# sijieaaa/AGPlace

Hardware: AMD Instinct MI355X
Metric: aerial-ground pairs/sec (backbone+ODE+pool) (higher is better)
Workload: dtype f16 (fp16 x fp16, fp32 accumulate); 1 GPU; nuScenes-AG 6-cam (C3/C4): MM.forward_q on [b,3,224,1344] + DBVanilla2D on [b,1,3,224,224], ResNet18 stem+layer1-3, euler h=0.1 x3 FCODE, GeM, stage-2 fusion; inference forward; the voxel branch's pooled outputs enter as fixed tensors (SURVEY.md 8d); global_batch=64, parallelism=dp1, bn=per-rank (eval: running statistics), paired_trunks=True, hipgraph=True, steps_in_flight=2, library_default_precision=4, headline_is_library_default=True, streams=2, query_sub_batches_on_streams=1, query_input=fp32 normalised panorama

## Files before the change

agplace_amd/csrc/stem_walk.hip:

```cpp
#include "conv_internal.hpp"

namespace agp_igemm {

[[maybe_unused]] constexpr int SWK_PROWB = 304;
[[maybe_unused]] constexpr int SWK_PROWS = 37;
constexpr int SWK_PBUF = 12 * 1024;
constexpr int SWK_EXCH = 2048;
constexpr int SWK_OFF_EXCH = 2 * SWK_PBUF;
constexpr int SWK_OFF_SS = SWK_OFF_EXCH + 2 * 4 * SWK_EXCH;
constexpr int SWK_OFF_STAGE = SWK_OFF_SS + 512;
constexpr int SWK_STAGE_W = 5 * 1024;
constexpr int SWK_OFF_W6 = SWK_OFF_STAGE + 4 * SWK_STAGE_W;
constexpr int SWK_OFF_LUT = SWK_OFF_W6 + 4096;
template <int IN> constexpr int swk_lds() { return IN == 2 ? SWK_OFF_LUT + 3 * 256 * 2 : (IN == 1 ? SWK_OFF_LUT : SWK_OFF_STAGE); }

struct WalkGeo {
    int nblk;
    int nseg, sps;
    int items, chunk;
    uint32_t o_bytes;
};

typedef __attribute__((ext_vector_type(4))) short s16x4;
__device__ __forceinline__ u32x2 pkmax4_h(const u32x2& a, const u32x2& b) {
    return __builtin_bit_cast(u32x2, __builtin_elementwise_max(__builtin_bit_cast(s16x4, a), __builtin_bit_cast(s16x4, b)));
}
__device__ __forceinline__ uint32_t pkmax2_h(uint32_t a, uint32_t b) {
    return __builtin_bit_cast(uint32_t, __builtin_elementwise_max(__builtin_bit_cast(s16x2, a), __builtin_bit_cast(s16x2, b)));
}
__device__ __forceinline__ uint32_t dpp_ror1(uint32_t v) { return (uint32_t)__builtin_amdgcn_mov_dpp((int)v, 0x121, 0xf, 0xf, true); }
__device__ __forceinline__ uint32_t dpp_shl1(uint32_t v) { return (uint32_t)__builtin_amdgcn_mov_dpp((int)v, 0x101, 0xf, 0xf, true); }
__device__ __forceinline__ uint32_t pack2_h_clamp(float a, float b, float hi) {
    const f32x2v v = {__builtin_amdgcn_fmed3f(a, 0.f, hi), __builtin_amdgcn_fmed3f(b, 0.f, hi)};
    return __builtin_bit_cast(uint32_t, __builtin_convertvector(v, f16x2));
}

template <int IN, class... RF>
__global__ void __launch_bounds__(256, 2) stem_walk_kernel(IgemmParams p, StemRaw raw, WalkGeo g, RF... rf) {
#if defined(__HIP_DEVICE_COMPILE__)
    constexpr bool RG = sizeof...(RF) != 0;
    extern __shared__ __attribute__((aligned(16))) char smem[];
    const int tid = threadIdx.x;
    const int lane = tid & 63;
    const int wave = __builtin_amdgcn_readfirstlane(tid >> 6);
    const int l15 = lane & 15, lq = lane >> 4;
    const int item = (blockIdx.x & 7) * g.chunk + (blockIdx.x >> 3);
    if (item >= g.items) return;
    const int seg = item % g.nseg;
    const int strip = item / g.nseg;
    const int pty = strip % p.pool_ty, pimg = strip / p.pool_ty;
    const int j0 = seg * g.sps, j1 = min(g.nblk, j0 + g.sps);
    const int js = j0 > 0 ? j0 - 1 : 0;
    const int oy0 = 14 * pty - 1;

    char* patch = smem;
    char* exch = smem + SWK_OFF_EXCH;
    float* ss = (float*)(smem + SWK_OFF_SS);
    if (tid < 64) {
        ss[tid] = p.scale ? p.scale[tid] : 1.f;
        ss[64 + tid] = p.shift ? p.shift[tid] : 0.f;
    }
    constexpr int WREG = IN >= 1 ? 6 : 7;
    bf16x8 wf[7][4];
    char* wl6 = smem + SWK_OFF_W6 + lane * 16;
#pragma unroll
    for (int ky = 0; ky < 7; ++ky)
#pragma unroll
        for (int nt = 0; nt < 4; ++nt) {
            const bf16x8 f = *(const bf16x8*)((const char*)p.w_hi + ((nt * 16 + l15) * p.Ktot + ky * 32 + lq * 8) * 2);
            if (ky < WREG) wf[ky][nt] = f;
            else *(bf16x8*)(wl6 + nt * 1024) = f;
        }

    const __amdgpu_buffer_rsrc_t rx = __builtin_amdgcn_make_buffer_rsrc((void*)p.x_hi, 0, p.x_bytes, 0x00020000);
    int choff[3];
    unsigned chok = 0;
    if constexpr (IN == 0) {
#pragma unroll
        for (int i = 0; i < 3; ++i) {
            const int c = (wave * 3 + i) * 64 + lane;
            const int pr = c / 19, pj = c - pr * 19;
            choff[i] = pr * p.x_sh * 2 + pj * 16;
            chok |= (pr < SWK_PROWS ? 1u : 0u) << i;
        }
    }
    const int xbase0 = (pimg * p.x_sn + 2 * oy0 * p.x_sh) * 2;

    auto issue_patch = [&](int j, int buf) {
        if constexpr (IN == 0) {
            const int base = xbase0 + 256 * j;
#pragma unroll
            for (int i = 0; i < 3; ++i) {
                const int off = ((chok >> i) & 1u) ? base + choff[i] : -16;
                __builtin_amdgcn_raw_ptr_buffer_load_lds(rx, LDS_PTR(patch + buf * SWK_PBUF + (wave * 3 + i) * 1024), 16, off, 0, 0, 0);
            }
        }
    };
    const __amdgpu_buffer_rsrc_t rraw = __builtin_amdgcn_make_buffer_rsrc((void*)raw.x, 0, raw.bytes, 0x00020000);
    char* stage = smem + SWK_OFF_STAGE + wave * SWK_STAGE_W;
    int rq[5];
    if constexpr (IN == 1) {
#pragma unroll
        for (int i = 0; i < 5; ++i) {
            const int q = i * 64 + lane;
            const int rr = q / 30, rem = q - rr * 30;
            const int ch = rem / 10, gq = rem - ch * 10;
            const int pr = wave + 4 * rr, iy = 2 * oy0 + pr - 3;
            const bool ok = q < 300 && pr < SWK_PROWS && iy >= 0 && iy < raw.h;
            const long long el = (long long)pimg * raw.sn + (long long)ch * raw.sc + (long long)iy * raw.sh + 4 * gq - 4;
            rq[i] = ok ? (int)(el * 4) | gq : -1;
        }
    }
    bf16_t* const lut = (bf16_t*)(smem + SWK_OFF_LUT);
    const int rowb = raw.wcam * 3;
    const int spc = raw.wcam >> 5;
    int riy[2];
    if constexpr (IN == 2) {
        for (int idx = tid; idx < 768; idx += 256) {
            const int c = idx >> 8, v = idx & 255;
            lut[idx] = f2h(((float)v / 255.f - raw.m[c]) / raw.s[c]);
        }
#pragma unroll
        for (int i = 0; i < 2; ++i) {
            const int rr = i * 8 + (lane >> 3);
            const int pr = wave + 4 * rr, iy = 2 * oy0 + pr - 3;
            riy[i] = (rr < 10 && pr < SWK_PROWS && iy >= 0 && iy < raw.h) ? iy * rowb : -1;
        }
        __syncthreads();
    }
    auto issue_raw = [&](int j) {
        if constexpr (IN == 2) {
            const int cam = j / spc, jj = j - cam * spc;
            const int img0 = pimg * raw.ncam;
            const int base_m = (img0 + cam) * raw.h * rowb + jj * 96;
            const bool lv = jj > 0 || cam > 0, rv = jj + 1 < spc || cam + 1 < raw.ncam;
            const int base_l = jj > 0 ? base_m - 16 : (img0 + cam - 1) * raw.h * rowb + rowb - 16;
            const int base_r = jj + 1 < spc ? base_m + 96 : (img0 + cam + 1) * raw.h * rowb;
            const int c8 = lane & 7;
            const int cb = c8 == 0 ? base_l : (c8 == 7 ? base_r : base_m + 16 * (c8 - 1));
            const bool cv = c8 == 0 ? lv : (c8 == 7 ? rv : true);
#pragma unroll
            for (int i = 0; i < 2; ++i) {
                const int off = (cv && riy[i] >= 0) ? cb + riy[i] : -16;
                __builtin_amdgcn_raw_ptr_buffer_load_lds(rraw, LDS_PTR(stage + i * 1024), 16, off, 0, 0, 0);
            }
        }
        if constexpr (IN == 1) {
#pragma unroll
            for (int i = 0; i < 5; ++i) {
                const int gq = rq[i] & 15;
                const int ix0 = 32 * j - 4 + 4 * gq;
                const bool ok = gq < 10 && ix0 >= 0 && ix0 < raw.w;
                const int off = ok ? (rq[i] & ~15) + 128 * j : -16;
                __builtin_amdgcn_raw_ptr_buffer_load_lds(rraw, LDS_PTR(stage + i * 1024), 16, off, 0, 0, 0);
            }
        }
    };
    RangeTrack<RG> rg;
    auto convert_raw = [&](int buf, int j) {
        if constexpr (IN == 2) {
#pragma unroll
            for (int t = 0; t < 6; ++t) {
                const int u = t * 64 + lane;
                const int rr = (u * 6899) >> 18, p_ = u - rr * 38;
                const int pr = wave + 4 * rr;
                if (u < 380 && pr < SWK_PROWS) {
                    const int iy = 2 * oy0 + pr - 3, col = 32 * j - 3 + p_;
                    const bool ok = iy >= 0 && iy < raw.h && col >= 0 && col < raw.w;
                    const int bo = rr * 128 + (p_ < 3 ? 7 + 3 * p_ : (p_ < 35 ? 16 + 3 * (p_ - 3) : 112 + 3 * (p_ - 35)));
                    const uint8_t* sb = (const uint8_t*)stage + bo;
                    const unsigned b0 = sb[0], b1 = sb[1], b2 = sb[2];
                    const bf16_t h0 = lut[b0], h1 = lut[256 + b1], h2 = lut[512 + b2];
                    const u32x2 pk = ok ? u32x2{pack2(h0, h1), pack2(h2, (bf16_t)0)} : u32x2{0u, 0u};
                    *(u32x2*)(patch + buf * SWK_PBUF + pr * SWK_PROWB + p_ * 8) = pk;
                }
            }
        }
        if constexpr (IN == 1) {
#pragma unroll
            for (int t = 0; t < 2; ++t) {
                const int u = t * 64 + lane;
                const int rr = u / 10, gq = u - rr * 10;
                const int pr = wave + 4 * rr;
                if (u < 100 && pr < SWK_PROWS) {
                    const char* sq = stage + (rr * 30 + gq) * 16;
                    const f32x4 c0 = *(const f32x4*)sq, c1 = *(const f32x4*)(sq + 160), c2 = *(const f32x4*)(sq + 320);
                    char* dst = patch + buf * SWK_PBUF + pr * SWK_PROWB + (4 * gq - 1) * 8;
#pragma unroll
                    for (int k = 0; k < 4; ++k) {
                        if ((gq == 0 && k == 0) || (gq == 9 && k == 3)) continue;
                        rg.sym2(c0[k], c1[k]);
                        rg.sym2(c2[k], 0.f);
                        *(u32x2*)(dst + k * 8) = u32x2{pack2(f2h(c0[k]), f2h(c1[k])), pack2(f2h(c2[k]), (bf16_t)0)};
                    }
                }
            }
        }
    };

    unsigned rowok = 0;
#pragma unroll
    for (int mt = 0; mt < 4; ++mt) {
        const int cy = oy0 + 4 * wave + mt;
        rowok |= ((cy >= 0 && cy < p.pool_h1) ? 1u : 0u) << mt;
    }
    const int pfo = (8 * wave) * SWK_PROWB + 16 * (l15 + lq);
    const int xo = lane * 16;
    const __amdgpu_buffer_rsrc_t ro = __builtin_amdgcn_make_buffer_rsrc(p.o_hi, 0, g.o_bytes, 0x00020000);
    const unsigned orow = (unsigned)(pimg * p.o_sn + p.o_base + 4 * lq) * 2u;

    uint32_t carry[2][4][2];
    u32x2 V[2][4];
#pragma unroll
    for (int r = 0; r < 2; ++r)
#pragma unroll
        for (int nt = 0; nt < 4; ++nt) { carry[r][nt][0] = 0u; carry[r][nt][1] = 0u; V[r][nt] = u32x2{0u, 0u}; }

    auto part2 = [&](int jj) {
        if (wave < 3) {
            const char* ex = exch + ((jj & 1) * 4 + wave + 1) * SWK_EXCH + xo;
            const u32x4 a = *(const u32x4*)ex, b = *(const u32x4*)(ex + 1024);
            V[1][0] = pkmax4_h(V[1][0], u32x2{a[0], a[1]});
            V[1][1] = pkmax4_h(V[1][1], u32x2{a[2], a[3]});
            V[1][2] = pkmax4_h(V[1][2], u32x2{b[0], b[1]});
            V[1][3] = pkmax4_h(V[1][3], u32x2{b[2], b[3]});
        }
        const bool first = l15 == 0;
        const int ox = 8 * jj + (l15 >> 1);
        const bool st = jj >= j0 && !(l15 & 1) && ox < p.pool_w2;
#pragma unroll
        for (int r = 0; r < 2; ++r) {
            const int oy = 7 * pty + 2 * wave + r;
            const bool str = st && oy < p.pool_h2 && (r == 0 || wave < 3);
            const unsigned off = str ? orow + (unsigned)(oy * p.o_sh + ox * p.o_sw) * 2u : 0xffffff00u;
#pragma unroll
            for (int nt = 0; nt < 4; ++nt) {
                u32x2 hm;
#pragma unroll
                for (int h = 0; h < 2; ++h) {
                    const uint32_t cur = V[r][nt][h];
                    const uint32_t rot = dpp_ror1(cur);
                    const uint32_t left = first ? carry[r][nt][h] : rot;
                    carry[r][nt][h] = rot;
                    hm[h] = pkmax2_h(pkmax2_h(left, cur), dpp_shl1(cur));
                }
                __builtin_amdgcn_raw_buffer_store_b64(hm, ro, off + nt * 32, 0, 0);
            }
        }
    };

    if constexpr (IN == 0) issue_patch(js, 0);
    else {
        issue_raw(js);
        asm volatile("s_waitcnt vmcnt(0)" ::: "memory");
        convert_raw(0, js);
    }
    for (int j = js; j < j1; ++j) {
        const int b = (j - js) & 1;
        if constexpr (IN == 0) {
            if (j <= js + 1) asm volatile("s_waitcnt vmcnt(0) lgkmcnt(0)" ::: "memory");
            else asm volatile("s_waitcnt vmcnt(8) lgkmcnt(0)" ::: "memory");
            __builtin_amdgcn_s_barrier();
        } else {
            asm volatile("s_waitcnt vmcnt(0) lgkmcnt(0)" ::: "memory");
            __syncthreads();
        }
        const bool more = j + 1 < j1;
        if (more) {
            if constexpr (IN == 0) issue_patch(j + 1, b ^ 1);
            else issue_raw(j + 1);
        }
        if (j > js) part2(j - 1);
        f32x4 acc[4][4];
        const char* pb = patch + b * SWK_PBUF + pfo;
#pragma unroll
        for (int ky = 0; ky < 7; ++ky) {
            bf16x8 xf[4];
#pragma unroll
            for (int mt = 0; mt < 4; ++mt) xf[mt] = *(const bf16x8*)(pb + (2 * mt + ky) * SWK_PROWB);
#pragma unroll
            for (int nt = 0; nt < 4; ++nt)
#pragma unroll
                for (int mt = 0; mt < 4; ++mt) {
                    if (ky == 0) acc[nt][mt] = f32x4{0.f, 0.f, 0.f, 0.f};
                    if (ky < WREG) {
                        mfma16<4>(acc[nt][mt], wf[ky][nt], wf[ky][nt], xf[mt], xf[mt]);
                    } else {
                        const bf16x8 w = *(const bf16x8*)(wl6 + nt * 1024);
                        mfma16<4>(acc[nt][mt], w, w, xf[mt], xf[mt]);
                    }
                }
        }
        const bool colok = 16 * j + l15 < p.pool_w1;
        float hi_[4];
#pragma unroll
        for (int mt = 0; mt < 4; ++mt) hi_[mt] = (colok && ((rowok >> mt) & 1u)) ? 65504.f : 0.f;
        u32x2 r0[4];
        RangeTrack<RG> rgm[4];
#pragma unroll
        for (int nt = 0; nt < 4; ++nt) {
            const f32x4 sc = *(const f32x4*)(ss + nt * 16 + 4 * lq), sh = *(const f32x4*)(ss + 64 + nt * 16 + 4 * lq);
            u32x2 r[4];
#pragma unroll
            for (int mt = 0; mt < 4; ++mt) {
                float v[4];
#pragma unroll
                for (int e = 0; e < 4; ++e) v[e] = acc[nt][mt][e] * sc[e] + sh[e];
                rgm[mt].pos2(v[0], v[1]);
                rgm[mt].pos2(v[2], v[3]);
                r[mt] = u32x2{pack2_h_clamp(v[0], v[1], hi_[mt]), pack2_h_clamp(v[2], v[3], hi_[mt])};
            }
            V[0][nt] = pkmax4_h(pkmax4_h(r[0], r[1]), r[2]);
            V[1][nt] = pkmax4_h(r[2], r[3]);
            r0[nt] = r[0];
        }
#pragma unroll
        for (int mt = 0; mt < 4; ++mt) rg.pos2(hi_[mt] > 0.f ? rgm[mt].hi : 0.f, 0.f);
        if (wave > 0) {
            char* ex = exch + ((j & 1) * 4 + wave) * SWK_EXCH + xo;
            *(u32x4*)ex = u32x4{r0[0][0], r0[0][1], r0[1][0], r0[1][1]};
            *(u32x4*)(ex + 1024) = u32x4{r0[2][0], r0[2][1], r0[3][0], r0[3][1]};
        }
        if constexpr (IN >= 1) {
            if (more) {
                asm volatile("s_waitcnt vmcnt(0)" ::: "memory");
                convert_raw(b ^ 1, j + 1);
            }
        }
    }
    asm volatile("s_waitcnt lgkmcnt(0)" ::: "memory");
    __syncthreads();
    part2(j1 - 1);
    rg.flush(rg_word(rf...), 0.f);
#endif
}

static WalkGeo walk_geo(int n, const IgemmParams& p) {
    WalkGeo g = {};
    g.nblk = (p.pool_w1 + 15) / 16;
    const long long strips = (long long)n * p.pool_ty;
    const int slots = 512;
    long long best = -1;
    for (int ns = 1; ns <= g.nblk && ns <= 32; ++ns) {
        const int sps = (g.nblk + ns - 1) / ns;
        const int nseg = (g.nblk + sps - 1) / sps;
        const long long rounds = (strips * nseg + slots - 1) / slots;
        const long long cost = rounds * (sps + (nseg > 1 ? 1 : 0) + 1);
        if (best < 0 || cost < best) { best = cost; g.nseg = nseg; g.sps = sps; }
    }
    g.items = (int)(strips * g.nseg);
    g.chunk = (g.items + 7) / 8;
    return g;
}

template <int IN, bool RG>
static int launch_stem_walk(IgemmParams& p, const StemRaw& raw, uint32_t* rflag, hipStream_t s) {
    constexpr int lds = swk_lds<IN>();
    static std::atomic<uint64_t> attr_done{0};
    if (!agp_lds_attr(RG ? (const void*)stem_walk_kernel<IN, uint32_t*> : (const void*)stem_walk_kernel<IN>, lds, attr_done))
        return AGP_E_LAUNCH;
    const int n = p.M / (p.pool_h1 * p.pool_w1);
    WalkGeo g = walk_geo(n, p);
    const long long o_bytes = (long long)n * p.o_sn * 2;
    if (o_bytes >= 0xffffff00ll) return AGP_E_BADARG;
    g.o_bytes = (uint32_t)o_bytes;
    if constexpr (RG) {
        AGP_LAUNCH((stem_walk_kernel<IN, uint32_t*>), dim3(g.chunk * 8), dim3(256), lds, s, p, raw, g, rflag);
    } else {
        (void)rflag;
        AGP_LAUNCH((stem_walk_kernel<IN>), dim3(g.chunk * 8), dim3(256), lds, s, p, raw, g);
    }
    AGP_CHECK_LAUNCH();
    return AGP_OK;
}

}

bool agp_internal_stem_walk_reads(const agp_igemm::StemRaw& raw, int n) {
    if (raw.sw != 1 || (raw.sn | raw.sc | raw.sh) % 4 || raw.w % 4 || ((uintptr_t)raw.x & 15)) return false;
    if (raw.sn < 0 || raw.sc < 0 || raw.sh < 0) return false;
    const long long last = (long long)(n - 1) * raw.sn + 2 * raw.sc + (long long)(raw.h - 1) * raw.sh + raw.w;
    return last * 4 < (1ll << 31);
}

bool agp_internal_stem_walk_reads_u8(const agp_igemm::StemRaw& raw, int n) {
    if (raw.wcam <= 0 || raw.wcam % 32 || raw.ncam <= 0 || raw.w != raw.ncam * raw.wcam || ((uintptr_t)raw.x & 15)) return false;
    return (long long)n * raw.ncam * raw.h * raw.wcam * 3 < (1ll << 31);
}

int agp_internal_stem_walk(agp_igemm::IgemmParams& p, int kind, agp_igemm::StemRaw raw, hipStream_t s) {
    using namespace agp_igemm;
    uint32_t* const rflag = agp_range_flag_get();
    if (kind == 0) return agp_rg_dispatch(rflag, [&](auto rg) { return launch_stem_walk<0, decltype(rg)::value>(p, raw, rflag, s); });
    if (kind == 2) {
        const int n = p.M / (p.pool_h1 * p.pool_w1);
        raw.bytes = (uint32_t)((long long)n * raw.ncam * raw.h * raw.wcam * 3);
        return agp_rg_dispatch(rflag, [&](auto rg) { return launch_stem_walk<2, decltype(rg)::value>(p, raw, rflag, s); });
    }
    if (kind == 1) {
        const int n = p.M / (p.pool_h1 * p.pool_w1);
        raw.bytes = (uint32_t)(((long long)(n - 1) * raw.sn + 2 * raw.sc + (long long)(raw.h - 1) * raw.sh + raw.w) * 4);
        return agp_rg_dispatch(rflag, [&](auto rg) { return launch_stem_walk<1, decltype(rg)::value>(p, raw, rflag, s); });
    }
    return AGP_E_BADARG;
}
```

Before: 42660 pairs/s.

## Max-pool raw accumulators before BN+ReLU in stem walk kernel

The stem conv epilogue used to apply BN scale/shift, ReLU and the fp16 pack to every output row before the vertical max-pool. It now pools the raw fp32 accumulators first, folding negative BN scales into sign flips and masking invalid rows with -FLT_MAX, so BN+ReLU runs only on the pooled rows in part2. The inter-wave exchange now carries fp32 instead of fp16, which doubles its LDS buffers, and the final part2 call is folded into the main loop. The intent is to cut VALU work in the epilogue, at the cost of more LDS traffic and footprint and a sign-flip pass whenever any scale is negative.

```diff
diff --git a/agplace_amd/csrc/stem_walk.hip b/agplace_amd/csrc/stem_walk.hip
--- a/agplace_amd/csrc/stem_walk.hip
+++ b/agplace_amd/csrc/stem_walk.hip
@@ -5,10 +5,10 @@
 [[maybe_unused]] constexpr int SWK_PROWB = 304;
 [[maybe_unused]] constexpr int SWK_PROWS = 37;
 constexpr int SWK_PBUF = 12 * 1024;
-constexpr int SWK_EXCH = 2048;
+constexpr int SWK_EXCH = 4096;
 constexpr int SWK_OFF_EXCH = 2 * SWK_PBUF;
-constexpr int SWK_OFF_SS = SWK_OFF_EXCH + 2 * 4 * SWK_EXCH;
-constexpr int SWK_OFF_STAGE = SWK_OFF_SS + 512;
+constexpr int SWK_OFF_SS = SWK_OFF_EXCH + 2 * 3 * SWK_EXCH;
+constexpr int SWK_OFF_STAGE = SWK_OFF_SS + 768;
 constexpr int SWK_STAGE_W = 5 * 1024;
 constexpr int SWK_OFF_W6 = SWK_OFF_STAGE + 4 * SWK_STAGE_W;
 constexpr int SWK_OFF_LUT = SWK_OFF_W6 + 4096;
@@ -21,18 +21,29 @@
     uint32_t o_bytes;
 };
 
-typedef __attribute__((ext_vector_type(4))) short s16x4;
-__device__ __forceinline__ u32x2 pkmax4_h(const u32x2& a, const u32x2& b) {
-    return __builtin_bit_cast(u32x2, __builtin_elementwise_max(__builtin_bit_cast(s16x4, a), __builtin_bit_cast(s16x4, b)));
-}
 __device__ __forceinline__ uint32_t pkmax2_h(uint32_t a, uint32_t b) {
     return __builtin_bit_cast(uint32_t, __builtin_elementwise_max(__builtin_bit_cast(s16x2, a), __builtin_bit_cast(s16x2, b)));
 }
 __device__ __forceinline__ uint32_t dpp_ror1(uint32_t v) { return (uint32_t)__builtin_amdgcn_mov_dpp((int)v, 0x121, 0xf, 0xf, true); }
 __device__ __forceinline__ uint32_t dpp_shl1(uint32_t v) { return (uint32_t)__builtin_amdgcn_mov_dpp((int)v, 0x101, 0xf, 0xf, true); }
-__device__ __forceinline__ uint32_t pack2_h_clamp(float a, float b, float hi) {
-    const f32x2v v = {__builtin_amdgcn_fmed3f(a, 0.f, hi), __builtin_amdgcn_fmed3f(b, 0.f, hi)};
-    return __builtin_bit_cast(uint32_t, __builtin_convertvector(v, f16x2));
+__device__ __forceinline__ float vmax3_f(float a, float b, float c) {
+    float d;
+    asm("v_max3_f32 %0, %1, %2, %3" : "=v"(d) : "v"(a), "v"(b), "v"(c));
+    return d;
+}
+__device__ __forceinline__ float vmax2_f(float a, float b) {
+    float d;
+    asm("v_max_f32 %0, %1, %2" : "=v"(d) : "v"(a), "v"(b));
+    return d;
+}
+template <class RT>
+__device__ __forceinline__ u32x2 bn_relu_h4(const f32x4& a, const f32x4& sc, const f32x4& sh, RT& rg) {
+    float v[4];
+#pragma unroll
+    for (int e = 0; e < 4; ++e) v[e] = __builtin_fmaf(a[e], sc[e], sh[e]);
+    rg.pos2(v[0], v[1]);
+    rg.pos2(v[2], v[3]);
+    return u32x2{pack2_h_lo(v[0], v[1], 0.f), pack2_h_lo(v[2], v[3], 0.f)};
 }
 
 template <int IN, class... RF>
@@ -56,10 +67,14 @@
     char* patch = smem;
     char* exch = smem + SWK_OFF_EXCH;
     float* ss = (float*)(smem + SWK_OFF_SS);
+    uint32_t* sgn = (uint32_t*)(smem + SWK_OFF_SS + 512);
     if (tid < 64) {
-        ss[tid] = p.scale ? p.scale[tid] : 1.f;
+        const uint32_t sb = p.scale ? __builtin_bit_cast(uint32_t, p.scale[tid]) : 0x3f800000u;
+        ss[tid] = __builtin_bit_cast(float, sb & 0x7fffffffu);
         ss[64 + tid] = p.shift ? p.shift[tid] : 0.f;
-    }
+        sgn[tid] = sb & 0x80000000u;
+    }
+    const bool negs = __builtin_amdgcn_ballot_w64(p.scale && (__builtin_bit_cast(uint32_t, p.scale[lane]) >> 31)) != 0;
     constexpr int WREG = IN >= 1 ? 6 : 7;
     bf16x8 wf[7][4];
     char* wl6 = smem + SWK_OFF_W6 + lane * 16;
@@ -210,41 +225,44 @@
     const unsigned orow = (unsigned)(pimg * p.o_sn + p.o_base + 4 * lq) * 2u;
 
     uint32_t carry[2][4][2];
-    u32x2 V[2][4];
+    f32x4 Vraw[2][4];
 #pragma unroll
     for (int r = 0; r < 2; ++r)
 #pragma unroll
-        for (int nt = 0; nt < 4; ++nt) { carry[r][nt][0] = 0u; carry[r][nt][1] = 0u; V[r][nt] = u32x2{0u, 0u}; }
+        for (int nt = 0; nt < 4; ++nt) { carry[r][nt][0] = 0u; carry[r][nt][1] = 0u; Vraw[r][nt] = f32x4{0.f, 0.f, 0.f, 0.f}; }
 
     auto part2 = [&](int jj) {
-        if (wave < 3) {
-            const char* ex = exch + ((jj & 1) * 4 + wave + 1) * SWK_EXCH + xo;
-            const u32x4 a = *(const u32x4*)ex, b = *(const u32x4*)(ex + 1024);
-            V[1][0] = pkmax4_h(V[1][0], u32x2{a[0], a[1]});
-            V[1][1] = pkmax4_h(V[1][1], u32x2{a[2], a[3]});
-            V[1][2] = pkmax4_h(V[1][2], u32x2{b[0], b[1]});
-            V[1][3] = pkmax4_h(V[1][3], u32x2{b[2], b[3]});
-        }
+        const char* ex = exch + ((jj & 1) * 3 + min(wave, 2)) * SWK_EXCH + xo;
         const bool first = l15 == 0;
         const int ox = 8 * jj + (l15 >> 1);
         const bool st = jj >= j0 && !(l15 & 1) && ox < p.pool_w2;
-#pragma unroll
-        for (int r = 0; r < 2; ++r) {
-            const int oy = 7 * pty + 2 * wave + r;
-            const bool str = st && oy < p.pool_h2 && (r == 0 || wave < 3);
-            const unsigned off = str ? orow + (unsigned)(oy * p.o_sh + ox * p.o_sw) * 2u : 0xffffff00u;
-#pragma unroll
-            for (int nt = 0; nt < 4; ++nt) {
+        const int oy = 7 * pty + 2 * wave;
+        const unsigned obase = orow + (unsigned)(oy * p.o_sh + ox * p.o_sw) * 2u;
+        unsigned orowb = (unsigned)p.o_sh * 2u;
+        asm volatile("" : "+s"(orowb));
+        unsigned off[2];
+        off[0] = (st && oy < p.pool_h2) ? obase : 0xffffff00u;
+        off[1] = (st && oy + 1 < p.pool_h2 && wave < 3) ? obase + orowb : 0xffffff00u;
+#pragma unroll
+        for (int nt = 0; nt < 4; ++nt) {
+            const f32x4 nb = *(const f32x4*)(ex + nt * 1024);
+            const f32x4 sc = *(const f32x4*)(ss + nt * 16 + 4 * lq), sh = *(const f32x4*)(ss + 64 + nt * 16 + 4 * lq);
+            f32x4 v1;
+#pragma unroll
+            for (int e = 0; e < 4; ++e) v1[e] = vmax2_f(Vraw[1][nt][e], nb[e]);
+            const u32x2 V[2] = {bn_relu_h4(Vraw[0][nt], sc, sh, rg), bn_relu_h4(v1, sc, sh, rg)};
+#pragma unroll
+            for (int r = 0; r < 2; ++r) {
                 u32x2 hm;
 #pragma unroll
                 for (int h = 0; h < 2; ++h) {
-                    const uint32_t cur = V[r][nt][h];
+                    const uint32_t cur = V[r][h];
                     const uint32_t rot = dpp_ror1(cur);
                     const uint32_t left = first ? carry[r][nt][h] : rot;
                     carry[r][nt][h] = rot;
                     hm[h] = pkmax2_h(pkmax2_h(left, cur), dpp_shl1(cur));
                 }
-                __builtin_amdgcn_raw_buffer_store_b64(hm, ro, off + nt * 32, 0, 0);
+                __builtin_amdgcn_raw_buffer_store_b64(hm, ro, off[r] + nt * 32, 0, 0);
             }
         }
     };
@@ -255,7 +273,7 @@
         asm volatile("s_waitcnt vmcnt(0)" ::: "memory");
         convert_raw(0, js);
     }
-    for (int j = js; j < j1; ++j) {
+    for (int j = js;; ++j) {
         const int b = (j - js) & 1;
         if constexpr (IN == 0) {
             if (j <= js + 1) asm volatile("s_waitcnt vmcnt(0) lgkmcnt(0)" ::: "memory");
@@ -271,6 +289,7 @@
             else issue_raw(j + 1);
         }
         if (j > js) part2(j - 1);
+        if (j == j1) break;
         f32x4 acc[4][4];
         const char* pb = patch + b * SWK_PBUF + pfo;
 #pragma unroll
@@ -291,35 +310,39 @@
                     }
                 }
         }
-        const bool colok = 16 * j + l15 < p.pool_w1;
-        float hi_[4];
-#pragma unroll
-        for (int mt = 0; mt < 4; ++mt) hi_[mt] = (colok && ((rowok >> mt) & 1u)) ? 65504.f : 0.f;
-        u32x2 r0[4];
-        RangeTrack<RG> rgm[4];
+        if (negs) {
+#pragma unroll
+            for (int nt = 0; nt < 4; ++nt) {
+                const u32x4 sg = *(const u32x4*)(sgn + nt * 16 + 4 * lq);
+#pragma unroll
+                for (int mt = 0; mt < 4; ++mt) acc[nt][mt] = __builtin_bit_cast(f32x4, __builtin_bit_cast(u32x4, acc[nt][mt]) ^ sg);
+            }
+        }
+        if (rowok != 15u || 16 * j + 16 > p.pool_w1) {
+            const bool colok = 16 * j + l15 < p.pool_w1;
+            float lose;
+            asm volatile("v_mov_b32 %0, 0xff7fffff" : "=v"(lose));
+#pragma unroll
+            for (int mt = 0; mt < 4; ++mt) {
+                const bool ok = colok && ((rowok >> mt) & 1u);
+#pragma unroll
+                for (int nt = 0; nt < 4; ++nt)
+#pragma unroll
+                    for (int e = 0; e < 4; ++e) acc[nt][mt][e] = ok ? acc[nt][mt][e] : lose;
+            }
+        }
 #pragma unroll
         for (int nt = 0; nt < 4; ++nt) {
-            const f32x4 sc = *(const f32x4*)(ss + nt * 16 + 4 * lq), sh = *(const f32x4*)(ss + 64 + nt * 16 + 4 * lq);
-            u32x2 r[4];
-#pragma unroll
-            for (int mt = 0; mt < 4; ++mt) {
-                float v[4];
-#pragma unroll
-                for (int e = 0; e < 4; ++e) v[e] = acc[nt][mt][e] * sc[e] + sh[e];
-                rgm[mt].pos2(v[0], v[1]);
-                rgm[mt].pos2(v[2], v[3]);
-                r[mt] = u32x2{pack2_h_clamp(v[0], v[1], hi_[mt]), pack2_h_clamp(v[2], v[3], hi_[mt])};
-            }
-            V[0][nt] = pkmax4_h(pkmax4_h(r[0], r[1]), r[2]);
-            V[1][nt] = pkmax4_h(r[2], r[3]);
-            r0[nt] = r[0];
-        }
-#pragma unroll
-        for (int mt = 0; mt < 4; ++mt) rg.pos2(hi_[mt] > 0.f ? rgm[mt].hi : 0.f, 0.f);
+#pragma unroll
+            for (int e = 0; e < 4; ++e) {
+                Vraw[0][nt][e] = vmax3_f(acc[nt][0][e], acc[nt][1][e], acc[nt][2][e]);
+                Vraw[1][nt][e] = vmax2_f(acc[nt][2][e], acc[nt][3][e]);
+            }
+        }
         if (wave > 0) {
-            char* ex = exch + ((j & 1) * 4 + wave) * SWK_EXCH + xo;
-            *(u32x4*)ex = u32x4{r0[0][0], r0[0][1], r0[1][0], r0[1][1]};
-            *(u32x4*)(ex + 1024) = u32x4{r0[2][0], r0[2][1], r0[3][0], r0[3][1]};
+            char* ex = exch + ((j & 1) * 3 + wave - 1) * SWK_EXCH + xo;
+#pragma unroll
+            for (int nt = 0; nt < 4; ++nt) *(f32x4*)(ex + nt * 1024) = acc[nt][0];
         }
         if constexpr (IN >= 1) {
             if (more) {
@@ -328,9 +351,6 @@
             }
         }
     }
-    asm volatile("s_waitcnt lgkmcnt(0)" ::: "memory");
-    __syncthreads();
-    part2(j1 - 1);
     rg.flush(rg_word(rf...), 0.f);
 #endif
 }
```

New measurement: 42790 pairs/s, median of 6. About the same (+0.3%).
